# CrossmodalGroup/DynamicVectorQuantization

Hardware: AMD Instinct MI355X
Metric: images/sec (256x256) DQ-VAE train step + VQ argmin GB/s, 1/2/4/8 MI355X (higher is better)
Workload: dtype bf16

## Files before the change

### dynamicvectorquantization_amd/_lib.py

```python
from __future__ import annotations

import ctypes as C
import os

HERE = os.path.dirname(os.path.abspath(__file__))
LIB_PATH = os.path.join(HERE, "libdvq_hip.so")

F32, BF16 = 0, 1
(IMPL_AUTO, IMPL_NAIVE, IMPL_MFMA, IMPL_REGSTAGE, IMPL_HALO, IMPL_WIDE, IMPL_WIDE_PIPE, IMPL_WIDE_PIPE_4WAVE, IMPL_WIDE_PIPE_192,
 IMPL_CONV_PIPE, IMPL_8PHASE) = range(11)

vp, i64, i32, f32, sz = C.c_void_p, C.c_int64, C.c_int32, C.c_float, C.c_size_t


class ConvDesc(C.Structure):
    _fields_ = [("N", i64), ("H", i64), ("W", i64), ("Cin", i64), ("OH", i64), ("OW", i64), ("Cout", i64),
                ("KH", i32), ("KW", i32), ("stride", i32), ("pad_t", i32), ("pad_l", i32), ("upsample", i32),
                ("dtype", i32), ("impl", i32)]


class DecodeLayer(C.Structure):
    _fields_ = [(n, vp) for n in ("wq", "wk", "wv", "wo", "w1", "w2", "bq", "bk", "bv", "bo", "b1", "b2", "ln1_g", "ln1_b", "ln2_g", "ln2_b",
                                  "kcache", "vcache")]

# ... 22 lines not shown

SCALAR_F32, SCALAR_BF16, SCALAR_F64, SCALAR_I32, SCALAR_I64, SCALAR_IMM, SCALAR_SKIP = range(7)
SCALAR_PUSH_MAX, SCALAR_COLUMNS_MAX = 64, 256


SIGNATURES = {
    "dvq_last_error": (C.c_char_p, []),
    "dvq_last_kernel": (C.c_char_p, []),
    "dvq_version": (i32, []),
    "dvq_check_device": (i32, []),
    "dvq_set_deterministic": (i32, [i32]),
    "dvq_deterministic": (i32, []),
    "dvq_unordered_launches": (C.c_longlong, []),
    "dvq_set_fp32_split": (i32, [i32]),
    "dvq_fp32_split": (i32, []),
    "dvq_probe_mfma_rate": (i32, [i32, vp, vp, vp]),
    "dvq_vq_prep_bytes": (sz, [i64, i64]),
    "dvq_vq_prepare": (i32, [vp, i64, i64, vp, vp]),
    "dvq_vq_argmin_workspace_bytes": (sz, [i64]),
    "dvq_vq_argmin": (i32, [vp, i32, vp, vp, i64, i64, i64, vp, vp, i32, vp]),
    "dvq_vq_distances": (i32, [vp, i32, vp, i64, i64, i64, vp, vp]),
    "dvq_vq_gather_loss": (i32, [vp, i32, vp, vp, vp, i64, i64, vp, vp, vp]),
    "dvq_vq_backward": (i32, [vp, vp, i32, vp, vp, vp, vp, i64, i64, vp, vp]),
    "dvq_vq_embed": (i32, [vp, vp, i64, i64, i32, vp, vp]),
    "dvq_vq_ema_stats": (i32, [vp, i32, vp, i64, i64, i64, vp, vp]),
    "dvq_vq_ema_apply": (i32, [vp, vp, f32, f32, i64, i64, vp, vp, vp, vp, vp]),
    "dvq_patch_entropy_gate": (i32, [vp, i64, i64, i64, i32, f32, vp, vp, vp]),
    "dvq_patch_entropy_gate_range": (i32, [vp, i64, i64, i64, i32, f32, f32, f32, vp, vp, vp]),
    "dvq_gn_stats": (i32, [vp, i32, i64, i64, i64, i32, vp, vp]),
    "dvq_gn_apply": (i32, [vp, i32, i64, i64, i64, i32, f32, vp, vp, vp, i32, vp, vp, vp]),
    "dvq_gn_bwd_partial_bytes": (sz, [i64, i64, i64]),
    "dvq_gn_bwd_reduce": (i32, [vp, vp, i32, i64, i64, i64, i32, vp, vp, vp, i32, vp, vp, vp, vp, vp]),
    "dvq_gn_bwd_dx": (i32, [vp, vp, i32, i64, i64, i64, i32, vp, vp, vp, i32, vp, vp, vp, vp]),
    "dvq_conv2d_fwd": (i32, [C.POINTER(ConvDesc), vp, vp, vp, vp, vp, vp, vp, i32, i32, vp]),
    "dvq_conv3x3_fused_ok": (i32, [C.POINTER(ConvDesc)]),
    "dvq_conv3x3_subpixel_ok": (i32, [C.POINTER(ConvDesc)]),
    "dvq_split_bf16_planes": (i32, [vp, vp, vp, i64, i64, i64, vp]),
    "dvq_conv3x3_x3_ok": (i32, [C.POINTER(ConvDesc), i32]),
    "dvq_conv3x3_x3_scratch_bytes": (i64, [C.POINTER(ConvDesc), i32]),
    "dvq_conv2d_fwd_x3": (i32, [C.POINTER(ConvDesc), vp, vp, vp, vp, vp, i32, vp, i64, vp]),
    "dvq_conv2d_dgrad_x3": (i32, [C.POINTER(ConvDesc), vp, vp, vp, vp, vp, i32, vp, i64, vp]),
    "dvq_conv2d_wgrad_x3_scratch_bytes": (i64, [C.POINTER(ConvDesc)]),
    "dvq_conv2d_wgrad_oihw_x3": (i32, [C.POINTER(ConvDesc), vp, vp, i64, i64, vp, vp, i32, vp, i64, vp]),
    "dvq_gn_scale_shift": (i32, [vp, vp, vp, i64, i64, i64, i32, f32, vp, vp, vp]),
    "dvq_conv2d_dgrad": (i32, [C.POINTER(ConvDesc), vp, vp, vp, vp, vp, i32, vp]),
    "dvq_set_workspace": (i32, [vp, i64]),
    "dvq_workspace_release": (i32, [vp]),
    "dvq_cmdlist_create": (i32, [vp, C.POINTER(vp)]),
    "dvq_cmdlist_replay": (i32, [vp, vp, vp]),
    "dvq_cmdlist_info": (i32, [vp, vp]),
    "dvq_cmdlist_destroy": (i32, [vp]),
    "dvq_permute_dual": (i32, [vp, vp, i64, i32, i32, i32, i64, i64, i64, i64, i64, i64, vp, vp, vp, vp, vp, vp]),
    "dvq_permute_dual_back": (i32, [vp, vp, vp, vp, i64, i64, i64, i32, i32, i64, i64, vp, vp]),
    "dvq_avgpool_slice": (i32, [vp, i32, i64, i64, i64, i64, i32, vp, i64, i64, vp]),
    "dvq_avgpool_slice_bwd": (i32, [vp, i32, i64, i64, i64, i64, i64, i64, i32, vp, vp]),
    "dvq_silu": (i32, [vp, i32, i64, vp, vp]),
    "dvq_silu_bwd": (i32, [vp, vp, i32, i64, vp, vp]),
    "dvq_relu": (i32, [vp, i32, i64, vp, vp]),
    "dvq_relu_bwd": (i32, [vp, vp, i32, i64, vp, vp]),
    "dvq_upsample_nearest2x": (i32, [vp, i32, i64, i64, i64, i64, vp, vp]),
    "dvq_upsample_nearest2x_bwd": (i32, [vp, i32, i64, i64, i64, i64, vp, vp]),
    "dvq_grain_merge": (i32, [vp, i32, vp, vp, i32, i64, i64, i64, i64, vp, vp, vp]),
    "dvq_grain_merge_bwd": (i32, [vp, vp, i32, vp, vp, i32, i64, i64, i64, i64, vp, vp, vp]),
    "dvq_affine_channels": (i32, [vp, i32, i64, i64, vp, vp, vp, vp]),
    "dvq_axpy_dev": (i32, [vp, vp, vp, i32, i64, vp, vp]),
    "dvq_maxpool2x2": (i32, [vp, i32, i64, i64, i64, i64, vp, vp]),
# ... 141 lines not shown
```

### dynamicvectorquantization_amd/csrc/groupnorm.hip

```cpp
#include "dvq_common.h"

#ifndef DVQ_GN_UNROLL
#define DVQ_GN_UNROLL 2
#endif

namespace {

__host__ __device__ inline int gn_rows_per_block(int64_t HW) { return HW > 4096 ? 1024 : 64; }

enum { ACT_NONE = 0, ACT_SILU = 1, ACT_LRELU = 2 };
template <int ACT>
__device__ __forceinline__ float act_fwd(float z) {
    if (ACT == ACT_SILU) return swishf(z);
    if (ACT == ACT_LRELU) return z > 0.f ? z : 0.2f * z;
    return z;
}
template <int ACT>
__device__ __forceinline__ float act_grad(float z) {
    if (ACT == ACT_SILU) return swish_grad(z);
    if (ACT == ACT_LRELU) return z > 0.f ? 1.f : 0.2f;
    return 1.f;
}

struct GnGeom {
    int ncol;
    int rows_per_pass;
    int cpg;
};

__device__ __forceinline__ GnGeom gn_geom(int64_t C, int G) {
    GnGeom g;
    g.ncol = (int)(C / 8);
    g.rows_per_pass = 256 / g.ncol;
    g.cpg = (int)(C / G);
    return g;
}

template <typename T, bool DET>
__global__ __launch_bounds__(256) void gn_stats_kernel(const T* __restrict__ x, int64_t HW, int64_t C, int G,
                                                       double* __restrict__ stats, int64_t rpb, double* __restrict__ part) {
    extern __shared__ __attribute__((aligned(16))) char smem[];
// ... 57 lines not shown
                dst[2 * g] += ds;
                dst[2 * g + 1] += dq;
            }
        }
    } else {
        for (int i = threadIdx.x; i < 2 * G; i += 256) atomicAdd(&stats[n * 2 * G + i], gs[i]);
    }
}

__device__ __forceinline__ void gn_mean_rstd(const double* stats, int64_t n, int G, int g, double cnt, float eps,
                                             float& mean, float& rstd) {
    const double m = stats[(n * G + g) * 2] / cnt;
    double var = stats[(n * G + g) * 2 + 1] / cnt - m * m;
    var = var < 0.0 ? 0.0 : var;
    mean = (float)m;
    rstd = (float)(1.0 / sqrt(var + (double)eps));
}

template <bool NT, typename T>
__device__ __forceinline__ void ld8(const T* p, float (&v)[8]) {
    if constexpr (NT) load8_nt(p, v);
    else load8(p, v);
}
template <bool NT, typename T>
__device__ __forceinline__ void st8(T* p, const float (&v)[8]) {
    if constexpr (NT) store8_nt(p, v);
    else store8(p, v);
}

template <typename T, int ACT, bool NT>
__global__ __launch_bounds__(256) void gn_apply_kernel(const T* __restrict__ x, int64_t HW, int64_t C, int G, float eps,
                                                       const double* __restrict__ stats,
                                                       const float* __restrict__ gamma, const float* __restrict__ beta,
                                                       T* __restrict__ y, float* __restrict__ mean_rstd) {
    extern __shared__ __attribute__((aligned(16))) char smem[];
    float* smr = reinterpret_cast<float*>(smem);
    const GnGeom ge = gn_geom(C, G);
    const int64_t n = blockIdx.y;
    const double cnt = (double)HW * ge.cpg;
    for (int g = threadIdx.x; g < G; g += 256) {
        float m, r;
        gn_mean_rstd(stats, n, G, g, cnt, eps, m, r);
        smr[2 * g] = m;
        smr[2 * g + 1] = r;
        if (blockIdx.x == 0 && mean_rstd != nullptr) {
            mean_rstd[(n * G + g) * 2] = m;
            mean_rstd[(n * G + g) * 2 + 1] = r;
        }
    }
    __syncthreads();
    const int col = threadIdx.x % ge.ncol, prow = threadIdx.x / ge.ncol;
    if (prow >= ge.rows_per_pass) return;
    float sc[8], sh[8];
#pragma unroll
    for (int j = 0; j < 8; ++j) {
        const int c = col * 8 + j, g = c / ge.cpg;
        sc[j] = smr[2 * g + 1] * gamma[c];
        sh[j] = beta[c] - smr[2 * g] * sc[j];
    }
    const int64_t p_end = min((int64_t)(blockIdx.x + 1) * gn_rows_per_block(HW), HW);
    const int64_t off = n * HW * C + col * 8;
    int64_t p = (int64_t)blockIdx.x * gn_rows_per_block(HW) + prow;
    const int64_t rpp = ge.rows_per_pass;
    for (; p + 3 * rpp < p_end; p += 4 * rpp) {
        float v[4][8];
#pragma unroll
        for (int u = 0; u < 4; ++u) ld8<NT>(x + off + (p + u * rpp) * C, v[u]);
#pragma unroll
        for (int u = 0; u < 4; ++u) {
#pragma unroll
            for (int j = 0; j < 8; ++j) v[u][j] = act_fwd<ACT>(fmaf(v[u][j], sc[j], sh[j]));
            st8<NT>(y + off + (p + u * rpp) * C, v[u]);
        }
    }
    for (; p < p_end; p += rpp) {
        float v[8];
        ld8<NT>(x + off + p * C, v);
#pragma unroll
        for (int j = 0; j < 8; ++j) {
            float z = fmaf(v[j], sc[j], sh[j]);
            v[j] = act_fwd<ACT>(z);
        }
        st8<NT>(y + off + p * C, v);
    }
}

template <typename T, int ACT, bool NT>
__global__ __launch_bounds__(256) void gn_bwd_reduce_kernel(const T* __restrict__ x, const T* __restrict__ dy,
                                                            int64_t HW, int64_t C, int G,
                                                            const float* __restrict__ mean_rstd,
                                                            const float* __restrict__ gamma,
                                                            const float* __restrict__ beta, double* __restrict__ red,
                                                            float* __restrict__ dgamma, float* __restrict__ dbeta,
                                                            float* __restrict__ part, int det) {
    extern __shared__ __attribute__((aligned(16))) char smem[];
    float* sA = reinterpret_cast<float*>(smem);
    float* sB = sA + C;
    const GnGeom ge = gn_geom(C, G);
    const int64_t n = blockIdx.y;
    for (int i = threadIdx.x; i < 2 * C; i += 256) sA[i] = 0.f;
    __syncthreads();
    const int col = threadIdx.x % ge.ncol, prow = threadIdx.x / ge.ncol;
    if (prow < ge.rows_per_pass) {
        float mu[8], rs[8], ga[8], be[8], a[8], b[8];
#pragma unroll
        for (int j = 0; j < 8; ++j) {
            const int c = col * 8 + j, g = c / ge.cpg;
            mu[j] = mean_rstd[(n * G + g) * 2];
            rs[j] = mean_rstd[(n * G + g) * 2 + 1];
            ga[j] = gamma[c];
            be[j] = beta[c];
            a[j] = b[j] = 0.f;
        }
        const int64_t p_end = min((int64_t)(blockIdx.x + 1) * gn_rows_per_block(HW), HW);
        const int64_t off = n * HW * C + col * 8;
        int64_t p = (int64_t)blockIdx.x * gn_rows_per_block(HW) + prow;
        const int64_t rpp = ge.rows_per_pass;
        auto accumulate = [&](const float (&v)[8], const float (&g8)[8]) {
#pragma unroll
            for (int j = 0; j < 8; ++j) {
                const float xh = (v[j] - mu[j]) * rs[j];
                float dz = g8[j];
                if (ACT != ACT_NONE) dz *= act_grad<ACT>(fmaf(xh, ga[j], be[j]));
                a[j] += dz;
                b[j] = fmaf(dz, xh, b[j]);
            }
        };
#if DVQ_GN_UNROLL > 1
        for (; p + rpp < p_end; p += 2 * rpp) {
            float v[2][8], g8[2][8];
#pragma unroll
            for (int u = 0; u < 2; ++u) {
                ld8<NT>(x + off + (p + u * rpp) * C, v[u]);
                ld8<NT>(dy + off + (p + u * rpp) * C, g8[u]);
            }
#pragma unroll
            for (int u = 0; u < 2; ++u) accumulate(v[u], g8[u]);
        }
#endif
        for (; p < p_end; p += rpp) {
            float v[8], g8[8];
            ld8<NT>(x + off + p * C, v);
            ld8<NT>(dy + off + p * C, g8);
            accumulate(v, g8);
        }
        if (det) {
            float* row = sA + (1 + prow) * 2 * C;
#pragma unroll
            for (int j = 0; j < 8; ++j) {
// ... 22 lines not shown
        for (int i = threadIdx.x; i < 2 * C; i += 256) dst[i] = sA[i];
        return;
    }
    for (int c = threadIdx.x; c < C; c += 256) {
        atomicAdd(&dbeta[c], sA[c]);
        atomicAdd(&dgamma[c], sB[c]);
    }
    for (int g = threadIdx.x; g < G; g += 256) {
        double s1 = 0.0, s2 = 0.0;
        for (int c = g * ge.cpg; c < (g + 1) * ge.cpg; ++c) {
            s1 += (double)gamma[c] * (double)sA[c];
            s2 += (double)gamma[c] * (double)sB[c];
        }
        atomicAdd(&red[(n * G + g) * 2], s1);
        atomicAdd(&red[(n * G + g) * 2 + 1], s2);
    }
}

__global__ __launch_bounds__(256) void gn_bwd_finalize_kernel(const float* __restrict__ part, int nb, int64_t C, int G,
                                                              const float* __restrict__ gamma, double* __restrict__ red,
                                                              float* __restrict__ dgamma, float* __restrict__ dbeta, int n_all,
                                                              float* __restrict__ img) {
    __shared__ double sm[4][64];
    const int rg = threadIdx.x >> 6, l = threadIdx.x & 63;
    const int ab = l >> 5, c = blockIdx.x * 32 + (l & 31);
    const int64_t n_lo = n_all > 0 ? 0 : blockIdx.y, n_hi = n_all > 0 ? n_all : blockIdx.y + 1;
    float dsum = 0.f;
    for (int64_t n = n_lo; n < n_hi; ++n) {
        double acc = 0.0;
        if (c < C) {
            const float* src = part + (int64_t)n * nb * 2 * C + ab * C + c;
            double a4[4] = {0.0, 0.0, 0.0, 0.0};
            int b = rg;
            for (; b + 12 < nb; b += 16) {
#pragma unroll
                for (int u = 0; u < 4; ++u) a4[u] += (double)src[(int64_t)(b + 4 * u) * 2 * C];
            }
            for (; b < nb; b += 4) a4[0] += (double)src[(int64_t)b * 2 * C];
            acc = (a4[0] + a4[1]) + (a4[2] + a4[3]);
        }
        __syncthreads();
        sm[rg][l] = acc;
        __syncthreads();
        if (rg != 0) continue;
        const double v = (sm[0][l] + sm[1][l]) + (sm[2][l] + sm[3][l]);
        if (n_all > 0) dsum += (float)v;
        else if (img != nullptr) {
            if (c < C) img[(n * 2 + ab) * C + c] = (float)v;
        } else if (c < C) atomicAdd(ab ? &dgamma[c] : &dbeta[c], (float)v);
        const int cpg = (int)(C / G);
        double w = c < C ? (double)gamma[c] * v : 0.0;
        for (int off = 1; off < cpg; off <<= 1) w += __shfl_xor(w, off, 64);
        if (c < C && (c & (cpg - 1)) == 0) red[(n * G + c / cpg) * 2 + ab] += w;
    }
    if (n_all > 0 && rg == 0 && c < C) (ab ? dgamma : dbeta)[c] += dsum;
}

template <typename T, int ACT, bool NT>
__global__ __launch_bounds__(256) void gn_bwd_dx_kernel(const T* __restrict__ x, const T* __restrict__ dy, int64_t HW,
                                                        int64_t C, int G, const float* __restrict__ mean_rstd,
                                                        const float* __restrict__ gamma, const float* __restrict__ beta,
                                                        const double* __restrict__ red, const T* __restrict__ addend,
                                                        T* __restrict__ dx) {
    extern __shared__ __attribute__((aligned(16))) char smem[];
    float* sm12 = reinterpret_cast<float*>(smem);
    const GnGeom ge = gn_geom(C, G);
    const int64_t n = blockIdx.y;
    const double cnt = (double)HW * ge.cpg;
    for (int g = threadIdx.x; g < G; g += 256) {
        sm12[2 * g] = (float)(red[(n * G + g) * 2] / cnt);
        sm12[2 * g + 1] = (float)(red[(n * G + g) * 2 + 1] / cnt);
    }
    __syncthreads();
    const int col = threadIdx.x % ge.ncol, prow = threadIdx.x / ge.ncol;
    if (prow >= ge.rows_per_pass) return;
    float mu[8], rs[8], ga[8], be[8], m1[8], m2[8];
#pragma unroll
    for (int j = 0; j < 8; ++j) {
        const int c = col * 8 + j, g = c / ge.cpg;
        mu[j] = mean_rstd[(n * G + g) * 2];
        rs[j] = mean_rstd[(n * G + g) * 2 + 1];
        ga[j] = gamma[c];
        be[j] = beta[c];
        m1[j] = sm12[2 * g];
        m2[j] = sm12[2 * g + 1];
    }
    const int64_t p_end = min((int64_t)(blockIdx.x + 1) * gn_rows_per_block(HW), HW);
    const int64_t off = n * HW * C + col * 8;
    int64_t p = (int64_t)blockIdx.x * gn_rows_per_block(HW) + prow;
    const int64_t rpp = ge.rows_per_pass;
    auto row_dx = [&](float (&v)[8], const float (&g8)[8]) {
#pragma unroll
        for (int j = 0; j < 8; ++j) {
            const float xh = (v[j] - mu[j]) * rs[j];
            float dz = g8[j];
            if (ACT != ACT_NONE) dz *= act_grad<ACT>(fmaf(xh, ga[j], be[j]));
            v[j] = rs[j] * (dz * ga[j] - m1[j] - xh * m2[j]);
        }
    };
#if DVQ_GN_UNROLL > 1
    for (; p + rpp < p_end; p += 2 * rpp) {
        float v[2][8], g8[2][8], ad[2][8];
#pragma unroll
        for (int u = 0; u < 2; ++u) {
            ld8<NT>(x + off + (p + u * rpp) * C, v[u]);
            ld8<NT>(dy + off + (p + u * rpp) * C, g8[u]);
            if (addend != nullptr) ld8<NT>(addend + off + (p + u * rpp) * C, ad[u]);
        }
#pragma unroll
        for (int u = 0; u < 2; ++u) {
            row_dx(v[u], g8[u]);
            if (addend != nullptr) {
#pragma unroll
                for (int j = 0; j < 8; ++j) v[u][j] += ad[u][j];
            }
            st8<NT>(dx + off + (p + u * rpp) * C, v[u]);
        }
    }
#endif
    for (; p < p_end; p += rpp) {
        float v[8], g8[8];
        ld8<NT>(x + off + p * C, v);
        ld8<NT>(dy + off + p * C, g8);
        row_dx(v, g8);
        if (addend != nullptr) {
            float ad[8];
            ld8<NT>(addend + off + p * C, ad);
#pragma unroll
            for (int j = 0; j < 8; ++j) v[j] += ad[j];
        }
        st8<NT>(dx + off + p * C, v);
    }
}

__global__ __launch_bounds__(256) void gn_scale_shift_kernel(const double* __restrict__ stats, const float* __restrict__ gamma,
                                                             const float* __restrict__ beta, int64_t N, int64_t C, int G,
                                                             double cnt, float eps, float* __restrict__ ss,
                                                             float* __restrict__ mean_rstd) {
    const int64_t e = (int64_t)blockIdx.x * 256 + threadIdx.x;
    if (e < N * C) {
        const int64_t n = e / C;
        const int c = (int)(e - n * C);
        float m, r;
        gn_mean_rstd(stats, n, G, c / (int)(C / G), cnt, eps, m, r);
        const float sc = r * gamma[c];
        ss[e * 2] = sc;
        ss[e * 2 + 1] = beta[c] - m * sc;
    }
    if (mean_rstd != nullptr && e < N * G) {
        float m, r;
        gn_mean_rstd(stats, e / G, G, (int)(e % G), cnt, eps, m, r);
        mean_rstd[e * 2] = m;
        mean_rstd[e * 2 + 1] = r;
    }
}

constexpr int64_t GN_STREAM_BYTES = 192ll << 20;

int gn_check(const char* who, int64_t N, int64_t HW, int64_t C, int G) {
    DVQ_REQUIRE(N > 0 && HW > 0 && C > 0 && G > 0 && C % G == 0 && C % 8 == 0 && C / 8 <= 256 && N <= 65535, DVQ_ESHAPE,
                "%s: unsupported shape N=%lld HW=%lld C=%lld G=%d", who, (long long)N, (long long)HW, (long long)C, G);
    return DVQ_OK;
}

}

extern "C" {

int dvq_gn_stats(const void* x, int dtype, int64_t N, int64_t HW, int64_t C, int G, double* stats,
                 dvq_stream_t stream) {
    DVQ_REQUIRE(x && stats, DVQ_EINVAL, "dvq_gn_stats: null pointer");
    if (int e = gn_check("dvq_gn_stats", N, HW, C, G)) return e;
    dim3 grid((unsigned)cdiv64(HW, gn_rows_per_block(HW)), (unsigned)N);
    hipStream_t s = (hipStream_t)stream;
    if (dvq_deterministic() != 0) {
        int64_t rpb = gn_rows_per_block(HW);
        const int64_t span = N * 2 * G;
        double* part = grid.x > 1 ? (double*)dvq_det_scratch(s, (int64_t)grid.x * span * 8) : nullptr;
        const int nb = (int)grid.x;
        if (part == nullptr) {
            rpb = HW;
            grid.x = 1;
        }
        const size_t lds = (2 * G + 256 * 8 * 2) * sizeof(double);
        DVQ_DISPATCH_DTYPE(dtype, T, gn_stats_kernel<T, true><<<grid, dim3(256), lds, s>>>((const T*)x, HW, C, G, stats, rpb, part););
        DVQ_CHECK_LAUNCH("gn_stats");
        if (part != nullptr) return dvq_det_fold_f64(stats, part, nb, span, span, s);
        return DVQ_OK;
    }
    dvq_note_unordered();
    DVQ_DISPATCH_DTYPE(dtype, T, gn_stats_kernel<T, false><<<grid, dim3(256), 2 * G * sizeof(double), s>>>(
                                     (const T*)x, HW, C, G, stats, (int64_t)gn_rows_per_block(HW), nullptr););
    DVQ_CHECK_LAUNCH("gn_stats");
    return DVQ_OK;
}

int dvq_gn_scale_shift(const double* stats, const float* gamma, const float* beta, int64_t N, int64_t HW, int64_t C, int G,
                       float eps, float* scale_shift, float* mean_rstd, dvq_stream_t stream) {
    DVQ_REQUIRE(stats && gamma && beta && scale_shift, DVQ_EINVAL, "dvq_gn_scale_shift: null pointer");
    if (int e = gn_check("dvq_gn_scale_shift", N, HW, C, G)) return e;
    const int64_t n = N * C > N * G ? N * C : N * G;
    gn_scale_shift_kernel<<<dim3((unsigned)cdiv64(n, 256)), dim3(256), 0, (hipStream_t)stream>>>(
        stats, gamma, beta, N, C, G, (double)HW * (double)(C / G), eps, scale_shift, mean_rstd);
    DVQ_CHECK_LAUNCH("gn_scale_shift");
    return DVQ_OK;
}

int dvq_gn_apply(const void* x, int dtype, int64_t N, int64_t HW, int64_t C, int G, float eps, const double* stats,
                 const float* gamma, const float* beta, int silu, void* y, float* mean_rstd, dvq_stream_t stream) {
    DVQ_REQUIRE(x && stats && gamma && beta && y, DVQ_EINVAL, "dvq_gn_apply: null pointer");
    if (int e = gn_check("dvq_gn_apply", N, HW, C, G)) return e;
    dim3 grid((unsigned)cdiv64(HW, gn_rows_per_block(HW)), (unsigned)N);
    hipStream_t s = (hipStream_t)stream;
#define GN_ACT_SWITCH_NT(KERN, NTV, LDS, ...)                                                           \
    if (silu == ACT_SILU) KERN<T, ACT_SILU, NTV><<<grid, dim3(256), LDS, s>>>(__VA_ARGS__);             \
    else if (silu == ACT_LRELU) KERN<T, ACT_LRELU, NTV><<<grid, dim3(256), LDS, s>>>(__VA_ARGS__);      \
    else KERN<T, ACT_NONE, NTV><<<grid, dim3(256), LDS, s>>>(__VA_ARGS__);
#define GN_ACT_SWITCH(KERN, LDS, ...)                                                                   \
    if (N * HW * C * (int64_t)sizeof(T) > GN_STREAM_BYTES) { GN_ACT_SWITCH_NT(KERN, true, LDS, __VA_ARGS__) } \
    else { GN_ACT_SWITCH_NT(KERN, false, LDS, __VA_ARGS__) }
    DVQ_DISPATCH_DTYPE(dtype, T, GN_ACT_SWITCH(gn_apply_kernel, 2 * G * sizeof(float), (const T*)x, HW, C, G, eps, stats, gamma, beta, (T*)y, mean_rstd));
    DVQ_CHECK_LAUNCH("gn_apply");
    return DVQ_OK;
}

size_t dvq_gn_bwd_partial_bytes(int64_t N, int64_t HW, int64_t C) {
    return (size_t)(N * cdiv64(HW, gn_rows_per_block(HW)) * 2 * C * (int64_t)sizeof(float));
}

int dvq_gn_bwd_reduce(const void* x, const void* dy, int dtype, int64_t N, int64_t HW, int64_t C, int G,
                      const float* mean_rstd, const float* gamma, const float* beta, int silu, double* red,
                      float* dgamma, float* dbeta, float* partials, dvq_stream_t stream) {
    DVQ_REQUIRE(x && dy && mean_rstd && gamma && beta && red && dgamma && dbeta, DVQ_EINVAL,
                "dvq_gn_bwd_reduce: null pointer");
    if (int e = gn_check("dvq_gn_bwd_reduce", N, HW, C, G)) return e;
    dim3 grid((unsigned)cdiv64(HW, gn_rows_per_block(HW)), (unsigned)N);
    hipStream_t s = (hipStream_t)stream;
    size_t lds = 2 * C * sizeof(float);
    const int64_t cpg = C / G;
    const bool fin_ok = (cpg & (cpg - 1)) == 0 && cpg <= 32;
    if (partials != nullptr && !fin_ok) partials = nullptr;
    const int det = dvq_deterministic() != 0 ? 1 : 0;
    float* img = nullptr;
    if (det) {
        DVQ_REQUIRE(fin_ok, DVQ_ESHAPE, "dvq_gn_bwd_reduce: deterministic mode needs a power-of-two C / G <= 32 (got %lld)", (long long)cpg);
        const int64_t pbytes = ((int64_t)dvq_gn_bwd_partial_bytes(N, HW, C) + 255) & ~(int64_t)255, ibytes = N * 2 * C * 4;
        if (partials == nullptr) {
            char* w = (char*)dvq_det_scratch(s, pbytes + ibytes);
            if (w == nullptr) w = (char*)dvq_det_scratch(s, pbytes);
            else img = (float*)(w + pbytes);
            partials = (float*)w;
        } else if (N > 1) {
            img = (float*)dvq_det_scratch(s, ibytes);
        }
        DVQ_REQUIRE(partials != nullptr, DVQ_EWORKSPACE, "dvq_gn_bwd_reduce: deterministic mode needs a partials buffer or a registered workspace");
        lds += (size_t)(256 / (C / 8)) * 2 * C * sizeof(float);
    } else {
        dvq_note_unordered();
    }
    DVQ_DISPATCH_DTYPE(dtype, T, GN_ACT_SWITCH(gn_bwd_reduce_kernel, lds, (const T*)x, (const T*)dy, HW, C, G, mean_rstd, gamma, beta, red, dgamma, dbeta, partials, det));
    DVQ_CHECK_LAUNCH("gn_bwd_reduce");
    if (partials != nullptr) {
        const bool serial = det && img == nullptr;
        gn_bwd_finalize_kernel<<<dim3((unsigned)cdiv64(C, 32), serial ? 1u : (unsigned)N), dim3(256), 0, s>>>(partials, (int)grid.x, C, G, gamma, red, dgamma, dbeta,
                                                                                                            serial ? (int)N : 0, img);
        DVQ_CHECK_LAUNCH("gn_bwd_finalize");
        if (img != nullptr) {
            if (int e = dvq_det_fold_f32(dbeta, img, (int)N, 2 * C, C, s)) return e;
            return dvq_det_fold_f32(dgamma, img + C, (int)N, 2 * C, C, s);
        }
    }
    return DVQ_OK;
}

int dvq_gn_bwd_dx(const void* x, const void* dy, int dtype, int64_t N, int64_t HW, int64_t C, int G,
                  const float* mean_rstd, const float* gamma, const float* beta, int silu, const double* red,
                  const void* addend, void* dx, dvq_stream_t stream) {
    DVQ_REQUIRE(x && dy && mean_rstd && gamma && beta && red && dx, DVQ_EINVAL, "dvq_gn_bwd_dx: null pointer");
    if (int e = gn_check("dvq_gn_bwd_dx", N, HW, C, G)) return e;
    dim3 grid((unsigned)cdiv64(HW, gn_rows_per_block(HW)), (unsigned)N);
    hipStream_t s = (hipStream_t)stream;
    DVQ_DISPATCH_DTYPE(dtype, T, GN_ACT_SWITCH(gn_bwd_dx_kernel, 2 * G * sizeof(float), (const T*)x, (const T*)dy, HW, C, G, mean_rstd, gamma, beta, red, (const T*)addend, (T*)dx));
    DVQ_CHECK_LAUNCH("gn_bwd_dx");
    return DVQ_OK;
}

}
```

### dynamicvectorquantization_amd/kernels.py

```python
from __future__ import annotations

import ctypes as C

import torch

from . import _lib
from . import runtime as rt
from ._lib import ConvDesc, check

_DT = {torch.float32: _lib.F32, torch.bfloat16: _lib.BF16}


def dt(t) -> int:
    d = t if isinstance(t, torch.dtype) else t.dtype
    if d not in _DT:
        raise TypeError(f"unsupported dtype {d}; libdvq_hip computes in float32 or bfloat16")
    return _DT[d]


def vec(dtype) -> int:
    return 4 if dtype == torch.float32 else 8


def _p(t):
# ... 304 lines not shown

def gn_stats(x, groups=32):
    n, c = x.shape[0], x.shape[-1]
    hw = x.numel() // (n * c)
    stats = zeros_small((n, groups, 2), torch.float64, x.device)
    check(lib().dvq_gn_stats(_p(x), dt(x), n, hw, c, groups, _p(stats), _s()), "dvq_gn_stats")
    return stats


def gn_forward(x, gamma, beta, groups=32, eps=1e-6, silu=True, stats=None):
    n, c = x.shape[0], x.shape[-1]
    hw = x.numel() // (n * c)
    if stats is None:
        stats = gn_stats(x, groups)
    y = torch.empty_like(x)
    mr = torch.empty(n, groups, 2, dtype=torch.float32, device=x.device)
    check(lib().dvq_gn_apply(_p(x), dt(x), n, hw, c, groups, eps, _p(stats), _p(gamma), _p(beta), int(silu), _p(y), _p(mr),
                             _s()), "dvq_gn_apply")
    return y, mr


def gn_scale_shift(x, gamma, beta, groups=32, eps=1e-6, stats=None):
    n, c = x.shape[0], x.shape[-1]
    hw = x.numel() // (n * c)
    if stats is None:
        stats = gn_stats(x, groups)
    ss = torch.empty(n, c, 2, dtype=torch.float32, device=x.device)
    mr = torch.empty(n, groups, 2, dtype=torch.float32, device=x.device)
    check(lib().dvq_gn_scale_shift(_p(stats), _p(gamma), _p(beta), n, hw, c, groups, eps, _p(ss), _p(mr), _s()),
          "dvq_gn_scale_shift")
    return ss, mr


def gn_backward(x, dy, mean_rstd, gamma, beta, dgamma, dbeta, groups=32, silu=True, addend=None, fixed_stats=False):
    n, c = x.shape[0], x.shape[-1]
    hw = x.numel() // (n * c)
    red = zeros_small((n, groups, 2), torch.float64, x.device)
    part = torch.empty(lib().dvq_gn_bwd_partial_bytes(n, hw, c), dtype=torch.uint8, device=x.device)
    check(lib().dvq_gn_bwd_reduce(_p(x), _p(dy), dt(x), n, hw, c, groups, _p(mean_rstd), _p(gamma), _p(beta), int(silu),
                                  _p(red), _p(dgamma), _p(dbeta), _p(part), _s()), "dvq_gn_bwd_reduce")
    if fixed_stats:
        red.zero_()
    dx = torch.empty_like(x)
    check(lib().dvq_gn_bwd_dx(_p(x), _p(dy), dt(x), n, hw, c, groups, _p(mean_rstd), _p(gamma), _p(beta), int(silu),
                              _p(red), _p(addend), _p(dx), _s()), "dvq_gn_bwd_dx")
    return dx


def conv_desc(n, h, w, cin, cout, kh, kw, stride, pad_t, pad_l, oh, ow, upsample, dtype, impl=0) -> ConvDesc:
    return ConvDesc(n, h, w, cin, oh, ow, cout, kh, kw, stride, pad_t, pad_l, int(upsample), dt(dtype), impl)


PACK_OHWI, PACK_SUBPIXEL = 256, 512


def subpixel_pack_views(wbuf, wtbuf, cout, cin):
    n9 = cout * 9 * cin
    return (wbuf[:n9].view(cout, 3, 3, cin), wtbuf[:n9].view(cin, 3, 3, cout), wbuf[n9:].view(4, cout, 4, cin),
            wtbuf[n9:].view(cin, 4, 4, cout))


def pack_weight(master_oihw, cin_p, cout_p, dtype, want_w=True, want_wt=True, subpixel=False):
    cout, cin, kh, kw = master_oihw.shape
    dev = master_oihw.device
    if subpixel:
        w = torch.empty(25 * cout * cin, dtype=dtype, device=dev)
        wt = torch.empty(25 * cout * cin, dtype=dtype, device=dev)
        check(lib().dvq_pack_weight(_p(master_oihw), cout, cin, kh, kw, cin_p, cout_p, dt(dtype) | PACK_SUBPIXEL, _p(w), _p(wt), _s()),
              "dvq_pack_weight")
# ... 1036 lines not shown
```

### include/dvq_hip.h

```cpp
#ifndef DVQ_HIP_H
#define DVQ_HIP_H

#include <stddef.h>
#include <stdint.h>

#ifdef __cplusplus
extern "C" {
#endif

typedef void* dvq_stream_t;
typedef void* dvq_cmdlist_t;

enum { DVQ_F32 = 0, DVQ_BF16 = 1 };
enum { DVQ_OK = 0, DVQ_EINVAL = -1, DVQ_ESHAPE = -2, DVQ_EARCH = -3, DVQ_ELAUNCH = -4, DVQ_EWORKSPACE = -5 };

const char* dvq_last_error(void);
const char* dvq_last_kernel(void);
int dvq_version(void);
int dvq_check_device(void);
int dvq_set_deterministic(int on);
int dvq_deterministic(void);
long long dvq_unordered_launches(void);
int dvq_set_fp32_split(int on);
int dvq_fp32_split(void);
// ... 8 lines not shown
                     dvq_stream_t stream);
int dvq_vq_argmin(const void* x, int x_dtype, const float* codebook, const void* prep, int64_t N, int64_t K,
                  int64_t D, int64_t* idx, void* ws, int impl, dvq_stream_t stream);

int dvq_vq_gather_loss(const void* x, int dtype, const float* codebook, const int64_t* idx, const float* mask,
                       int64_t N, int64_t D, void* x_q, double* loss_sum, dvq_stream_t stream);
int dvq_vq_backward(const void* g_xq, const void* x, int dtype, const float* codebook, const int64_t* idx,
                    const float* mask, const float* coef_dev, int64_t N, int64_t D, void* dx, dvq_stream_t stream);
int dvq_vq_embed(const float* codebook, const int64_t* idx, int64_t N, int64_t D, int out_dtype, void* out,
                 dvq_stream_t stream);

int dvq_vq_ema_stats(const void* x, int dtype, const int64_t* idx, int64_t N, int64_t K, int64_t D, float* stats,
                     dvq_stream_t stream);
int dvq_vq_ema_apply(const float* stats, const float* restart_rows, float decay, float eps, int64_t K, int64_t D,
                     float* cluster_size_ema, float* embed_ema, float* weight, float* scratch_sum,
                     dvq_stream_t stream);

int dvq_patch_entropy_gate(const float* img, int64_t B, int64_t H, int64_t W, int patch, float threshold,
                           float* entropy, int64_t* gate, dvq_stream_t stream);
int dvq_patch_entropy_gate_range(const float* img, int64_t B, int64_t H, int64_t W, int patch, float bin_lo, float bin_hi,
                                 float threshold, float* entropy, int64_t* gate, dvq_stream_t stream);

int dvq_gn_stats(const void* x, int dtype, int64_t N, int64_t HW, int64_t C, int G, double* stats,
                 dvq_stream_t stream);
int dvq_gn_apply(const void* x, int dtype, int64_t N, int64_t HW, int64_t C, int G, float eps, const double* stats,
                 const float* gamma, const float* beta, int silu, void* y, float* mean_rstd, dvq_stream_t stream);
size_t dvq_gn_bwd_partial_bytes(int64_t N, int64_t HW, int64_t C);
int dvq_gn_bwd_reduce(const void* x, const void* dy, int dtype, int64_t N, int64_t HW, int64_t C, int G,
                      const float* mean_rstd, const float* gamma, const float* beta, int silu, double* red,
                      float* dgamma, float* dbeta, float* partials, dvq_stream_t stream);
int dvq_gn_bwd_dx(const void* x, const void* dy, int dtype, int64_t N, int64_t HW, int64_t C, int G,
                  const float* mean_rstd, const float* gamma, const float* beta, int silu, const double* red,
                  const void* addend, void* dx, dvq_stream_t stream);

enum {
    DVQ_IMPL_AUTO = 0,
    DVQ_IMPL_NAIVE = 1,
    DVQ_IMPL_MFMA = 2,
    DVQ_IMPL_REGSTAGE = 3,
    DVQ_IMPL_HALO = 4,
    DVQ_IMPL_WIDE = 5,
    DVQ_IMPL_WIDE_PIPE = 6,
    DVQ_IMPL_WIDE_PIPE_4WAVE = 7,
    DVQ_IMPL_WIDE_PIPE_192 = 8,
    DVQ_IMPL_CONV_PIPE = 9,
    DVQ_IMPL_8PHASE = 10
};

typedef struct dvq_conv_desc {
    int64_t N;
    int64_t H, W;
    int64_t Cin;
    int64_t OH, OW;
    int64_t Cout;
    int32_t KH, KW;
    int32_t stride;
    int32_t pad_t, pad_l;
    int32_t upsample;
    int32_t dtype;
    int32_t impl;
} dvq_conv_desc;

enum { DVQ_ACT_NONE = 0, DVQ_ACT_SWISH = 1, DVQ_ACT_LRELU = 2, DVQ_ACT_RELU = 3 };

int dvq_conv3x3_fused_ok(const dvq_conv_desc* d);
int dvq_conv3x3_subpixel_ok(const dvq_conv_desc* d);
// ... 280 lines not shown
```

Measured before the change: 457.7.

## Add one-pass register-resident GroupNorm backward and size-aware row-per-block tuning

Adds a fused GroupNorm backward kernel for bf16 with small spatial extents (HW up to 1024). Each block keeps a 64-channel slab of x and dy in registers, reduces dgamma/dbeta and the group means in-block, then writes dx without reading the inputs a second time. This replaces the two-kernel reduce + dx path and its partial buffer whenever the shape allows. It also makes rows-per-block for the stats, apply, reduce and dx passes depend on tensor size and grid fill, and unrolls the partial-sum fold further. The fused kernel uses many registers per thread and adds a deterministic-fold path, which costs extra launches when deterministic mode is on.

```diff
diff --git a/dynamicvectorquantization_amd/_lib.py b/dynamicvectorquantization_amd/_lib.py
--- a/dynamicvectorquantization_amd/_lib.py
+++ b/dynamicvectorquantization_amd/_lib.py
@@ -78,6 +78,8 @@
     "dvq_gn_bwd_partial_bytes": (sz, [i64, i64, i64]),
     "dvq_gn_bwd_reduce": (i32, [vp, vp, i32, i64, i64, i64, i32, vp, vp, vp, i32, vp, vp, vp, vp, vp]),
     "dvq_gn_bwd_dx": (i32, [vp, vp, i32, i64, i64, i64, i32, vp, vp, vp, i32, vp, vp, vp, vp]),
+    "dvq_gn_bwd_onepass_ok": (i32, [i32, i64, i64, i64, i32, vp]),
+    "dvq_gn_backward": (i32, [vp, vp, i32, i64, i64, i64, i32, vp, vp, vp, i32, i32, vp, vp, vp, vp, vp]),
     "dvq_conv2d_fwd": (i32, [C.POINTER(ConvDesc), vp, vp, vp, vp, vp, vp, vp, i32, i32, vp]),
     "dvq_conv3x3_fused_ok": (i32, [C.POINTER(ConvDesc)]),
     "dvq_conv3x3_subpixel_ok": (i32, [C.POINTER(ConvDesc)]),
diff --git a/dynamicvectorquantization_amd/csrc/groupnorm.hip b/dynamicvectorquantization_amd/csrc/groupnorm.hip
--- a/dynamicvectorquantization_amd/csrc/groupnorm.hip
+++ b/dynamicvectorquantization_amd/csrc/groupnorm.hip
@@ -6,7 +6,24 @@
 
 namespace {
 
-__host__ __device__ inline int gn_rows_per_block(int64_t HW) { return HW > 4096 ? 1024 : 64; }
+#ifndef DVQ_GN_ROWS
+#define DVQ_GN_ROWS 64, 64, 512, 64
+#endif
+#ifndef DVQ_GN_FILL
+#define DVQ_GN_FILL 256, 512, 256, 512
+#endif
+enum { GN_STATS = 0, GN_APPLY = 1, GN_REDUCE = 2, GN_DX = 3 };
+constexpr int GN_SMALL_ROWS[4] = {DVQ_GN_ROWS};
+constexpr int GN_FILL_BLOCKS[4] = {DVQ_GN_FILL};
+constexpr int64_t GN_GEOM_ELEMS = 4ll << 20;
+
+inline int gn_rows_per_block(int pass, int64_t N, int64_t HW, int64_t C) {
+    int rpb = HW > 4096 ? 1024 : 64;
+    if (N * HW * C < GN_GEOM_ELEMS) return rpb;
+    if (HW <= 4096) rpb = GN_SMALL_ROWS[pass];
+    while (rpb > 64 && N * cdiv64(HW, rpb) < GN_FILL_BLOCKS[pass]) rpb >>= 1;
+    return rpb;
+}
 
 enum { ACT_NONE = 0, ACT_SILU = 1, ACT_LRELU = 2 };
 template <int ACT>
@@ -130,7 +147,7 @@
 __global__ __launch_bounds__(256) void gn_apply_kernel(const T* __restrict__ x, int64_t HW, int64_t C, int G, float eps,
                                                        const double* __restrict__ stats,
                                                        const float* __restrict__ gamma, const float* __restrict__ beta,
-                                                       T* __restrict__ y, float* __restrict__ mean_rstd) {
+                                                       T* __restrict__ y, float* __restrict__ mean_rstd, int rpb) {
     extern __shared__ __attribute__((aligned(16))) char smem[];
     float* smr = reinterpret_cast<float*>(smem);
     const GnGeom ge = gn_geom(C, G);
@@ -156,9 +173,9 @@
         sc[j] = smr[2 * g + 1] * gamma[c];
         sh[j] = beta[c] - smr[2 * g] * sc[j];
     }
-    const int64_t p_end = min((int64_t)(blockIdx.x + 1) * gn_rows_per_block(HW), HW);
+    const int64_t p_end = min((int64_t)(blockIdx.x + 1) * rpb, HW);
     const int64_t off = n * HW * C + col * 8;
-    int64_t p = (int64_t)blockIdx.x * gn_rows_per_block(HW) + prow;
+    int64_t p = (int64_t)blockIdx.x * rpb + prow;
     const int64_t rpp = ge.rows_per_pass;
     for (; p + 3 * rpp < p_end; p += 4 * rpp) {
         float v[4][8];
@@ -190,7 +207,7 @@
                                                             const float* __restrict__ gamma,
                                                             const float* __restrict__ beta, double* __restrict__ red,
                                                             float* __restrict__ dgamma, float* __restrict__ dbeta,
-                                                            float* __restrict__ part, int det) {
+                                                            float* __restrict__ part, int det, int rpb) {
     extern __shared__ __attribute__((aligned(16))) char smem[];
     float* sA = reinterpret_cast<float*>(smem);
     float* sB = sA + C;
@@ -210,9 +227,9 @@
             be[j] = beta[c];
             a[j] = b[j] = 0.f;
         }
-        const int64_t p_end = min((int64_t)(blockIdx.x + 1) * gn_rows_per_block(HW), HW);
+        const int64_t p_end = min((int64_t)(blockIdx.x + 1) * rpb, HW);
         const int64_t off = n * HW * C + col * 8;
-        int64_t p = (int64_t)blockIdx.x * gn_rows_per_block(HW) + prow;
+        int64_t p = (int64_t)blockIdx.x * rpb + prow;
         const int64_t rpp = ge.rows_per_pass;
         auto accumulate = [&](const float (&v)[8], const float (&g8)[8]) {
 #pragma unroll
@@ -301,6 +318,13 @@
             const float* src = part + (int64_t)n * nb * 2 * C + ab * C + c;
             double a4[4] = {0.0, 0.0, 0.0, 0.0};
             int b = rg;
+            for (; b + 60 < nb; b += 64) {
+                float t[16];
+#pragma unroll
+                for (int u = 0; u < 16; ++u) t[u] = src[(int64_t)(b + 4 * u) * 2 * C];
+#pragma unroll
+                for (int u = 0; u < 16; ++u) a4[u & 3] += (double)t[u];
+            }
             for (; b + 12 < nb; b += 16) {
 #pragma unroll
                 for (int u = 0; u < 4; ++u) a4[u] += (double)src[(int64_t)(b + 4 * u) * 2 * C];
@@ -330,7 +354,7 @@
                                                         int64_t C, int G, const float* __restrict__ mean_rstd,
                                                         const float* __restrict__ gamma, const float* __restrict__ beta,
                                                         const double* __restrict__ red, const T* __restrict__ addend,
-                                                        T* __restrict__ dx) {
+                                                        T* __restrict__ dx, int rpb) {
     extern __shared__ __attribute__((aligned(16))) char smem[];
     float* sm12 = reinterpret_cast<float*>(smem);
     const GnGeom ge = gn_geom(C, G);
@@ -354,9 +378,9 @@
         m1[j] = sm12[2 * g];
         m2[j] = sm12[2 * g + 1];
     }
-    const int64_t p_end = min((int64_t)(blockIdx.x + 1) * gn_rows_per_block(HW), HW);
+    const int64_t p_end = min((int64_t)(blockIdx.x + 1) * rpb, HW);
     const int64_t off = n * HW * C + col * 8;
-    int64_t p = (int64_t)blockIdx.x * gn_rows_per_block(HW) + prow;
+    int64_t p = (int64_t)blockIdx.x * rpb + prow;
     const int64_t rpp = ge.rows_per_pass;
     auto row_dx = [&](float (&v)[8], const float (&g8)[8]) {
 #pragma unroll
@@ -399,6 +423,144 @@
             for (int j = 0; j < 8; ++j) v[j] += ad[j];
         }
         st8<NT>(dx + off + p * C, v);
+    }
+}
+
+constexpr int GN1_SLAB = 64, GN1_THREADS = 512, GN1_PASS = GN1_THREADS / 8, GN1_MAX_ROWS = 16;
+constexpr int64_t GN1_MAX_HW = (int64_t)GN1_MAX_ROWS * GN1_PASS;
+constexpr int64_t GN1_MIN_BLOCKS = 128;
+
+__device__ __forceinline__ void unpack8(const uint4& a, float (&v)[8]) {
+    v[0] = __uint_as_float(a.x << 16); v[1] = __uint_as_float(a.x & 0xffff0000u);
+    v[2] = __uint_as_float(a.y << 16); v[3] = __uint_as_float(a.y & 0xffff0000u);
+    v[4] = __uint_as_float(a.z << 16); v[5] = __uint_as_float(a.z & 0xffff0000u);
+    v[6] = __uint_as_float(a.w << 16); v[7] = __uint_as_float(a.w & 0xffff0000u);
+}
+
+template <int ACT, int ROWS, bool PERCH>
+__global__ __launch_bounds__(GN1_THREADS) void gn_bwd_onepass_kernel(const bf16_t* __restrict__ x, const bf16_t* __restrict__ dy, int HW,
+                                                                     int C, int G, const float* __restrict__ mean_rstd,
+                                                                     const float* __restrict__ gamma, const float* __restrict__ beta,
+                                                                     const bf16_t* __restrict__ addend, bf16_t* __restrict__ dx,
+                                                                     float* __restrict__ dgamma, float* __restrict__ dbeta,
+                                                                     float* __restrict__ img, int det, int fixed) {
+    __shared__ float sW[GN1_THREADS / 64][2][GN1_SLAB];
+    __shared__ float sMR[2][GN1_SLAB];
+    __shared__ float sM[2][GN1_SLAB];
+    const int tid = threadIdx.x, col = tid & 7, prow = tid >> 3, wave = tid >> 6, lane = tid & 63;
+    const int n = blockIdx.y, c0 = blockIdx.x * GN1_SLAB;
+    const int cpg = C / G, cpg_shift = __ffs(cpg) - 1;
+    const int64_t base = (int64_t)n * HW * C + c0;
+    const bf16_t* xb = x + base;
+    const bf16_t* gb = dy + base;
+    const unsigned off = (unsigned)(prow * C + col * 8), step = (unsigned)(GN1_PASS * C);
+    uint4 xr[ROWS], gr[ROWS];
+#pragma unroll
+    for (int u = 0; u < ROWS; ++u) {
+        const int p = prow + u * GN1_PASS;
+        xr[u] = gr[u] = make_uint4(0u, 0u, 0u, 0u);
+        if (p < HW) {
+            xr[u] = *reinterpret_cast<const uint4*>(xb + (off + u * step));
+            gr[u] = *reinterpret_cast<const uint4*>(gb + (off + u * step));
+        }
+    }
+    if (tid < GN1_SLAB) {
+        const int g = (c0 + tid) >> cpg_shift;
+        sMR[0][tid] = mean_rstd[((int64_t)n * G + g) * 2];
+        sMR[1][tid] = mean_rstd[((int64_t)n * G + g) * 2 + 1];
+    }
+    float ga[8], be[8];
+#pragma unroll
+    for (int j = 0; j < 8; ++j) {
+        ga[j] = gamma[c0 + col * 8 + j];
+        be[j] = beta[c0 + col * 8 + j];
+    }
+    __syncthreads();
+    constexpr int NP = PERCH ? 8 : 1;
+    float mu[NP], rs[NP], a[8], b[8];
+#pragma unroll
+    for (int j = 0; j < NP; ++j) {
+        mu[j] = sMR[0][col * 8 + j];
+        rs[j] = sMR[1][col * 8 + j];
+    }
+#pragma unroll
+    for (int j = 0; j < 8; ++j) a[j] = b[j] = 0.f;
+#pragma unroll
+    for (int u = 0; u < ROWS; ++u) {
+        if (prow + u * GN1_PASS < HW) {
+            float v[8], g8[8];
+            unpack8(xr[u], v);
+            unpack8(gr[u], g8);
+#pragma unroll
+            for (int j = 0; j < 8; ++j) {
+                const float xh = (v[j] - mu[PERCH ? j : 0]) * rs[PERCH ? j : 0];
+                float dz = g8[j];
+                if (ACT != ACT_NONE) dz *= act_grad<ACT>(fmaf(xh, ga[j], be[j]));
+                a[j] += dz;
+                b[j] = fmaf(dz, xh, b[j]);
+            }
+        }
+    }
+#pragma unroll
+    for (int u = 0; u < ROWS; ++u) {
+        asm volatile("" : "+v"(xr[u].x), "+v"(xr[u].y), "+v"(xr[u].z), "+v"(xr[u].w));
+        asm volatile("" : "+v"(gr[u].x), "+v"(gr[u].y), "+v"(gr[u].z), "+v"(gr[u].w));
+    }
+#pragma unroll
+    for (int j = 0; j < 8; ++j) {
+#pragma unroll
+        for (int o = 8; o < 64; o <<= 1) {
+            a[j] += __shfl_xor(a[j], o, 64);
+            b[j] += __shfl_xor(b[j], o, 64);
+        }
+    }
+    if (lane < 8) {
+#pragma unroll
+        for (int j = 0; j < 8; ++j) {
+            sW[wave][0][col * 8 + j] = a[j];
+            sW[wave][1][col * 8 + j] = b[j];
+        }
+    }
+    __syncthreads();
+    if (tid < 2 * GN1_SLAB) {
+        const int ab = tid >> 6, c = c0 + lane;
+        float t = 0.f;
+#pragma unroll
+        for (int w = 0; w < GN1_THREADS / 64; ++w) t += sW[w][ab][lane];
+        if (!det) atomicAdd(ab ? &dgamma[c] : &dbeta[c], t);
+        else if (img != nullptr) img[((int64_t)n * 2 + ab) * C + c] = t;
+        else (ab ? dgamma : dbeta)[c] += t;
+        double w = (double)gamma[c] * (double)t;
+        for (int o = 1; o < cpg; o <<= 1) w += __shfl_xor(w, o, 64);
+        if ((lane & (cpg - 1)) == 0) sM[ab][lane >> cpg_shift] = fixed ? 0.f : (float)(w / ((double)HW * cpg));
+    }
+    __syncthreads();
+    float m1[NP], m2[NP];
+#pragma unroll
+    for (int j = 0; j < NP; ++j) {
+        m1[j] = sM[0][(col * 8 + j) >> cpg_shift];
+        m2[j] = sM[1][(col * 8 + j) >> cpg_shift];
+    }
+#pragma unroll
+    for (int u = 0; u < ROWS; ++u) {
+        const int p = prow + u * GN1_PASS;
+        if (p < HW) {
+            uint4 ar = make_uint4(0u, 0u, 0u, 0u);
+            if (addend != nullptr) ar = *reinterpret_cast<const uint4*>(addend + base + (off + u * step));
+            float v[8], g8[8], ad[8];
+            unpack8(xr[u], v);
+            unpack8(gr[u], g8);
+            unpack8(ar, ad);
+#pragma unroll
+            for (int j = 0; j < 8; ++j) {
+                const float xh = (v[j] - mu[PERCH ? j : 0]) * rs[PERCH ? j : 0];
+                float dz = g8[j];
+                if (ACT != ACT_NONE) dz *= act_grad<ACT>(fmaf(xh, ga[j], be[j]));
+                v[j] = rs[PERCH ? j : 0] * (dz * ga[j] - m1[PERCH ? j : 0] - xh * m2[PERCH ? j : 0]);
+                if (addend != nullptr) v[j] += ad[j];
+            }
+            store8(dx + base + (off + u * step), v);
+        }
     }
 }
 
@@ -432,18 +594,74 @@
     return DVQ_OK;
 }
 
+bool gn_onepass_runs(int dtype, int64_t N, int64_t HW, int64_t C, int G) {
+    if (dtype != DVQ_BF16 || N <= 0 || N > 65535 || HW <= 0 || HW > GN1_MAX_HW || G <= 0 || C <= 0 || C % G != 0 || C % GN1_SLAB != 0 || C > 2048) return false;
+    const int64_t cpg = C / G;
+    return (cpg & (cpg - 1)) == 0 && cpg <= 32;
+}
+
 }
 
 extern "C" {
+
+int dvq_gn_bwd_onepass_ok(int dtype, int64_t N, int64_t HW, int64_t C, int G, dvq_stream_t stream) {
+    if (!gn_onepass_runs(dtype, N, HW, C, G) || N * (C / GN1_SLAB) < GN1_MIN_BLOCKS) return 0;
+    if (dvq_deterministic() != 0 && N > 1 && dvq_det_scratch((hipStream_t)stream, N * 2 * C * 4) == nullptr) return 0;
+    return 1;
+}
+
+int dvq_gn_backward(const void* x, const void* dy, int dtype, int64_t N, int64_t HW, int64_t C, int G, const float* mean_rstd,
+                    const float* gamma, const float* beta, int silu, int fixed_stats, const void* addend, void* dx, float* dgamma,
+                    float* dbeta, dvq_stream_t stream) {
+    DVQ_REQUIRE(x && dy && mean_rstd && gamma && beta && dx && dgamma && dbeta, DVQ_EINVAL, "dvq_gn_backward: null pointer");
+    DVQ_REQUIRE(gn_onepass_runs(dtype, N, HW, C, G), DVQ_ESHAPE,
+                "dvq_gn_backward: the one-pass kernel takes bf16, HW <= %lld, C %% %d == 0 and a power-of-two C / G <= 32 (got dtype %d N=%lld HW=%lld C=%lld G=%d)",
+                (long long)GN1_MAX_HW, GN1_SLAB, dtype, (long long)N, (long long)HW, (long long)C, G);
+    DVQ_REQUIRE(silu == ACT_NONE || silu == ACT_SILU || silu == ACT_LRELU, DVQ_EINVAL, "dvq_gn_backward: activation code %d", silu);
+    hipStream_t s = (hipStream_t)stream;
+    const int det = dvq_deterministic() != 0 ? 1 : 0;
+    float* img = nullptr;
+    if (det && N > 1) {
+        img = (float*)dvq_det_scratch(s, N * 2 * C * 4);
+        DVQ_REQUIRE(img != nullptr, DVQ_EWORKSPACE, "dvq_gn_backward: deterministic mode with N > 1 needs a registered workspace");
+    }
+    if (!det && N > 1) dvq_note_unordered();
+    const dim3 grid((unsigned)(C / GN1_SLAB), (unsigned)N);
+#define GN1_LAUNCH(A, R, P)                                                                                                              \
+    gn_bwd_onepass_kernel<A, R, P><<<grid, dim3(GN1_THREADS), 0, s>>>((const bf16_t*)x, (const bf16_t*)dy, (int)HW, (int)C, G, mean_rstd, gamma, \
+                                                                   beta, (const bf16_t*)addend, (bf16_t*)dx, dgamma, dbeta, img, det, fixed_stats)
+#define GN1_ROWS_SWITCH(A, P)                                \
+    if (HW <= 1 * GN1_PASS) GN1_LAUNCH(A, 1, P);             \
+    else if (HW <= 2 * GN1_PASS) GN1_LAUNCH(A, 2, P);        \
+    else if (HW <= 4 * GN1_PASS) GN1_LAUNCH(A, 4, P);        \
+    else if (HW <= 8 * GN1_PASS) GN1_LAUNCH(A, 8, P);        \
+    else GN1_LAUNCH(A, 16, P);
+#define GN1_ACT_SWITCH(P)                                               \
+    if (silu == ACT_SILU) { GN1_ROWS_SWITCH(ACT_SILU, P) }              \
+    else if (silu == ACT_LRELU) { GN1_ROWS_SWITCH(ACT_LRELU, P) }       \
+    else { GN1_ROWS_SWITCH(ACT_NONE, P) }
+    if (C / G < 8) { GN1_ACT_SWITCH(true) }
+    else { GN1_ACT_SWITCH(false) }
+#undef GN1_ACT_SWITCH
+#undef GN1_ROWS_SWITCH
+#undef GN1_LAUNCH
+    DVQ_CHECK_LAUNCH("gn_bwd_onepass");
+    if (img != nullptr) {
+        if (int e = dvq_det_fold_f32(dbeta, img, (int)N, 2 * C, C, s)) return e;
+        return dvq_det_fold_f32(dgamma, img + C, (int)N, 2 * C, C, s);
+    }
+    return DVQ_OK;
+}
 
 int dvq_gn_stats(const void* x, int dtype, int64_t N, int64_t HW, int64_t C, int G, double* stats,
                  dvq_stream_t stream) {
     DVQ_REQUIRE(x && stats, DVQ_EINVAL, "dvq_gn_stats: null pointer");
     if (int e = gn_check("dvq_gn_stats", N, HW, C, G)) return e;
-    dim3 grid((unsigned)cdiv64(HW, gn_rows_per_block(HW)), (unsigned)N);
+    const int rows = gn_rows_per_block(GN_STATS, N, HW, C);
+    dim3 grid((unsigned)cdiv64(HW, rows), (unsigned)N);
     hipStream_t s = (hipStream_t)stream;
     if (dvq_deterministic() != 0) {
-        int64_t rpb = gn_rows_per_block(HW);
+        int64_t rpb = rows;
         const int64_t span = N * 2 * G;
         double* part = grid.x > 1 ? (double*)dvq_det_scratch(s, (int64_t)grid.x * span * 8) : nullptr;
         const int nb = (int)grid.x;
@@ -459,7 +677,7 @@
     }
     dvq_note_unordered();
     DVQ_DISPATCH_DTYPE(dtype, T, gn_stats_kernel<T, false><<<grid, dim3(256), 2 * G * sizeof(double), s>>>(
-                                     (const T*)x, HW, C, G, stats, (int64_t)gn_rows_per_block(HW), nullptr););
+                                     (const T*)x, HW, C, G, stats, (int64_t)rows, nullptr););
     DVQ_CHECK_LAUNCH("gn_stats");
     return DVQ_OK;
 }
@@ -479,7 +697,8 @@
                  const float* gamma, const float* beta, int silu, void* y, float* mean_rstd, dvq_stream_t stream) {
     DVQ_REQUIRE(x && stats && gamma && beta && y, DVQ_EINVAL, "dvq_gn_apply: null pointer");
     if (int e = gn_check("dvq_gn_apply", N, HW, C, G)) return e;
-    dim3 grid((unsigned)cdiv64(HW, gn_rows_per_block(HW)), (unsigned)N);
+    const int rows = gn_rows_per_block(GN_APPLY, N, HW, C);
+    dim3 grid((unsigned)cdiv64(HW, rows), (unsigned)N);
     hipStream_t s = (hipStream_t)stream;
 #define GN_ACT_SWITCH_NT(KERN, NTV, LDS, ...)                                                           \
     if (silu == ACT_SILU) KERN<T, ACT_SILU, NTV><<<grid, dim3(256), LDS, s>>>(__VA_ARGS__);             \
@@ -488,13 +707,13 @@
 #define GN_ACT_SWITCH(KERN, LDS, ...)                                                                   \
     if (N * HW * C * (int64_t)sizeof(T) > GN_STREAM_BYTES) { GN_ACT_SWITCH_NT(KERN, true, LDS, __VA_ARGS__) } \
     else { GN_ACT_SWITCH_NT(KERN, false, LDS, __VA_ARGS__) }
-    DVQ_DISPATCH_DTYPE(dtype, T, GN_ACT_SWITCH(gn_apply_kernel, 2 * G * sizeof(float), (const T*)x, HW, C, G, eps, stats, gamma, beta, (T*)y, mean_rstd));
+    DVQ_DISPATCH_DTYPE(dtype, T, GN_ACT_SWITCH(gn_apply_kernel, 2 * G * sizeof(float), (const T*)x, HW, C, G, eps, stats, gamma, beta, (T*)y, mean_rstd, rows));
     DVQ_CHECK_LAUNCH("gn_apply");
     return DVQ_OK;
 }
 
 size_t dvq_gn_bwd_partial_bytes(int64_t N, int64_t HW, int64_t C) {
-    return (size_t)(N * cdiv64(HW, gn_rows_per_block(HW)) * 2 * C * (int64_t)sizeof(float));
+    return (size_t)(N * cdiv64(HW, gn_rows_per_block(GN_REDUCE, N, HW, C)) * 2 * C * (int64_t)sizeof(float));
 }
 
 int dvq_gn_bwd_reduce(const void* x, const void* dy, int dtype, int64_t N, int64_t HW, int64_t C, int G,
@@ -503,7 +722,8 @@
     DVQ_REQUIRE(x && dy && mean_rstd && gamma && beta && red && dgamma && dbeta, DVQ_EINVAL,
                 "dvq_gn_bwd_reduce: null pointer");
     if (int e = gn_check("dvq_gn_bwd_reduce", N, HW, C, G)) return e;
-    dim3 grid((unsigned)cdiv64(HW, gn_rows_per_block(HW)), (unsigned)N);
+    const int rows = gn_rows_per_block(GN_REDUCE, N, HW, C);
+    dim3 grid((unsigned)cdiv64(HW, rows), (unsigned)N);
     hipStream_t s = (hipStream_t)stream;
     size_t lds = 2 * C * sizeof(float);
     const int64_t cpg = C / G;
@@ -527,7 +747,7 @@
     } else {
         dvq_note_unordered();
     }
-    DVQ_DISPATCH_DTYPE(dtype, T, GN_ACT_SWITCH(gn_bwd_reduce_kernel, lds, (const T*)x, (const T*)dy, HW, C, G, mean_rstd, gamma, beta, red, dgamma, dbeta, partials, det));
+    DVQ_DISPATCH_DTYPE(dtype, T, GN_ACT_SWITCH(gn_bwd_reduce_kernel, lds, (const T*)x, (const T*)dy, HW, C, G, mean_rstd, gamma, beta, red, dgamma, dbeta, partials, det, rows));
     DVQ_CHECK_LAUNCH("gn_bwd_reduce");
     if (partials != nullptr) {
         const bool serial = det && img == nullptr;
@@ -547,9 +767,10 @@
                   const void* addend, void* dx, dvq_stream_t stream) {
     DVQ_REQUIRE(x && dy && mean_rstd && gamma && beta && red && dx, DVQ_EINVAL, "dvq_gn_bwd_dx: null pointer");
     if (int e = gn_check("dvq_gn_bwd_dx", N, HW, C, G)) return e;
-    dim3 grid((unsigned)cdiv64(HW, gn_rows_per_block(HW)), (unsigned)N);
+    const int rows = gn_rows_per_block(GN_DX, N, HW, C);
+    dim3 grid((unsigned)cdiv64(HW, rows), (unsigned)N);
     hipStream_t s = (hipStream_t)stream;
-    DVQ_DISPATCH_DTYPE(dtype, T, GN_ACT_SWITCH(gn_bwd_dx_kernel, 2 * G * sizeof(float), (const T*)x, (const T*)dy, HW, C, G, mean_rstd, gamma, beta, red, (const T*)addend, (T*)dx));
+    DVQ_DISPATCH_DTYPE(dtype, T, GN_ACT_SWITCH(gn_bwd_dx_kernel, 2 * G * sizeof(float), (const T*)x, (const T*)dy, HW, C, G, mean_rstd, gamma, beta, red, (const T*)addend, (T*)dx, rows));
     DVQ_CHECK_LAUNCH("gn_bwd_dx");
     return DVQ_OK;
 }
diff --git a/dynamicvectorquantization_amd/kernels.py b/dynamicvectorquantization_amd/kernels.py
--- a/dynamicvectorquantization_amd/kernels.py
+++ b/dynamicvectorquantization_amd/kernels.py
@@ -360,9 +360,20 @@
     return ss, mr
 
 
+def gn_backward_onepass(x, dy, mean_rstd, gamma, beta, dgamma, dbeta, groups=32, silu=True, addend=None, fixed_stats=False):
+    n, c = x.shape[0], x.shape[-1]
+    hw = x.numel() // (n * c)
+    dx = torch.empty_like(x)
+    check(lib().dvq_gn_backward(_p(x), _p(dy), dt(x), n, hw, c, groups, _p(mean_rstd), _p(gamma), _p(beta), int(silu),
+                                int(bool(fixed_stats)), _p(addend), _p(dx), _p(dgamma), _p(dbeta), _s()), "dvq_gn_backward")
+    return dx
+
+
 def gn_backward(x, dy, mean_rstd, gamma, beta, dgamma, dbeta, groups=32, silu=True, addend=None, fixed_stats=False):
     n, c = x.shape[0], x.shape[-1]
     hw = x.numel() // (n * c)
+    if lib().dvq_gn_bwd_onepass_ok(dt(x), n, hw, c, groups, _s()):
+        return gn_backward_onepass(x, dy, mean_rstd, gamma, beta, dgamma, dbeta, groups, silu, addend, fixed_stats)
     red = zeros_small((n, groups, 2), torch.float64, x.device)
     part = torch.empty(lib().dvq_gn_bwd_partial_bytes(n, hw, c), dtype=torch.uint8, device=x.device)
     check(lib().dvq_gn_bwd_reduce(_p(x), _p(dy), dt(x), n, hw, c, groups, _p(mean_rstd), _p(gamma), _p(beta), int(silu),
diff --git a/include/dvq_hip.h b/include/dvq_hip.h
--- a/include/dvq_hip.h
+++ b/include/dvq_hip.h
@@ -64,6 +64,11 @@
 int dvq_gn_bwd_dx(const void* x, const void* dy, int dtype, int64_t N, int64_t HW, int64_t C, int G,
                   const float* mean_rstd, const float* gamma, const float* beta, int silu, const double* red,
                   const void* addend, void* dx, dvq_stream_t stream);
+
+int dvq_gn_bwd_onepass_ok(int dtype, int64_t N, int64_t HW, int64_t C, int G, dvq_stream_t stream);
+int dvq_gn_backward(const void* x, const void* dy, int dtype, int64_t N, int64_t HW, int64_t C, int G, const float* mean_rstd,
+                    const float* gamma, const float* beta, int silu, int fixed_stats, const void* addend, void* dx, float* dgamma,
+                    float* dbeta, dvq_stream_t stream);
 
 enum {
     DVQ_IMPL_AUTO = 0,
```

Result: no change. 461.6, median of 6 (+0.9%).
